# discord/lilliput

Hardware: NVIDIA H100
Metric: images_per_sec_1080p_jpeg_to_256x256_jpeg_q85 (higher is better)
Workload: dtype u8

## Files before the change

### lilliput_b200/csrc/abi_opencv.cu

```cuda
#include <algorithm>
#include <cstring>
#include <memory>
#include <mutex>
#include <new>
#include <string>
#include <vector>

#include "common.cuh"
#include "kernels.cuh"
#include "lp_opencv.h"

namespace lp {

thread_local long g_launches = 0;

static std::once_flag g_dev_once;
static int g_dev_status = LP_ERR_CUDA;

int ensure_device() {
    std::call_once(g_dev_once, [] {
        int n = 0;
        cudaError_t e = cudaGetDeviceCount(&n);
        if (e != cudaSuccess || n == 0) {
            fprintf(stderr,
// ... 99 lines not shown
    m->type = type;
    m->step = row;
    m->dev_off = 0;
    m->dev_step = row;
    m->is_view = false;
    m->dev_valid = true;
    m->host_valid = false;
    return LP_OK;
}

struct Decoder {
    const uint8_t* data = nullptr;
    size_t len = 0;
    JpegHeader jpeg;
    PngHeader png;
    bool is_png = false;
    bool header_ok = false;
    std::string description;
};

struct Encoder {
    std::string ext;
    Mat* dst = nullptr;
};

static int sync_stream() {
    LP_CUDA_OK(cudaStreamSynchronize(thread_stream()));
    return LP_OK;
}

static int decode_jpeg_into(const Decoder* d, Mat* m) {
    const JpegHeader& h = d->jpeg;
    if (!h.supported && !h.multiscan) {
        fprintf(stderr, "[lilliput_b200] JPEG variant not supported on the device path (sampling layout)\n");
        return LP_ERR_UNSUPPORTED;
    }
    std::vector<JpegScanDesc> scans;
    std::vector<JpegHuffSet> sets(1);
    int nscans = 0, nsets = 1;
    if (h.multiscan) {
        scans.resize(kMultiscanMaxScans);
        sets.resize(kMultiscanMaxSets);
        int rc = jpeg_parse_scans(d->data, d->len, h, scans.data(), (int)scans.size(), &nscans, sets.data(),
                                  (int)sets.size(), &nsets);
        if (rc) return rc;
        const size_t visits = jpeg_multiscan_visits(h, scans.data(), nscans);
        if (visits > kMultiscanMaxVisits) {
            fprintf(stderr, "[lilliput_b200] multi-scan JPEG: %zu block visits over %d scans exceed the serial decoder's budget\n",
                    visits, nscans);
            return LP_ERR_UNSUPPORTED;
        }
    } else {
        jpeg_build_huff_set(h, &sets[0]);
        if (h.restart_interval) {
            scans.resize(1);
            jpeg_baseline_scan(h, &scans[0]);
            nscans = 1;
        }
    }
    const bool parallel = nscans == 0;
    cudaStream_t st = thread_stream();
    JpegDecodeItem it;
    memset(&it, 0, sizeof(it));
    it.scan_off = 0;
    it.scan_len = (uint32_t)h.scan_length;
    it.table_set = 0;
    it.restart_interval = h.restart_interval;
    const uint32_t total_blocks = jpeg_decode_item(h, &it);
    uint32_t tiles = 0;
    const uint32_t blocks = jpeg_item_set_window(&it, 0, 0, h.width, h.height, false, &tiles);
    if (!parallel) {
        it.restart_interval = 0;
        it.table_set = 0;
        it.nscans = (uint32_t)nscans;
    }

    uint8_t* scratch = nullptr;
    const size_t upload_len = parallel ? h.scan_length : d->len;
    const size_t scan_bytes = round_up(upload_len + 16, (size_t)256);
    const size_t sets_b = round_up(sizeof(JpegHuffSet) * (size_t)nsets, (size_t)256);
    const size_t scans_b = round_up(sizeof(JpegScanDesc) * (size_t)nscans + 16, (size_t)256);
    const size_t coef_bytes = round_up((size_t)blocks * 64 * sizeof(int16_t), (size_t)256);
    const size_t clean_b = parallel ? round_up(huff_clean_bytes(h.scan_length), (size_t)256) : 0;
    const size_t states_b = parallel ? round_up(2 * huff_nsub(h.scan_length) * 8, (size_t)256) : 0;
    const size_t nslots_b = parallel ? round_up(2 * huff_nsub(h.scan_length) * 4, (size_t)256) : 0;
    const size_t dcdiff_b = parallel ? round_up((size_t)total_blocks * 2, (size_t)256) : 0;
    const size_t total = 1024 + sets_b + scan_bytes + coef_bytes + clean_b + states_b + nslots_b +
                         dcdiff_b + scans_b;
    LP_CUDA_OK(cudaMallocAsync(&scratch, total, st));
    JpegDecodeItem* d_item = reinterpret_cast<JpegDecodeItem*>(scratch);
    JpegHuffSet* d_hs = reinterpret_cast<JpegHuffSet*>(scratch + 1024);
    uint8_t* d_scan = scratch + 1024 + sets_b;
    int16_t* d_coef = reinterpret_cast<int16_t*>(d_scan + scan_bytes);
    uint8_t* d_clean = reinterpret_cast<uint8_t*>(d_coef) + coef_bytes;
    uint8_t* d_states = d_clean + clean_b;
    uint8_t* d_nslots = d_states + states_b;
    uint8_t* d_dcdiff = d_nslots + nslots_b;
    JpegScanDesc* d_scans = reinterpret_cast<JpegScanDesc*>(d_dcdiff + dcdiff_b);
    LP_CUDA_OK(cudaMemcpyAsync(d_item, &it, sizeof(it), cudaMemcpyHostToDevice, st));
    LP_CUDA_OK(cudaMemcpyAsync(d_hs, sets.data(), sizeof(JpegHuffSet) * nsets, cudaMemcpyHostToDevice, st));
    if (parallel) {
        LP_CUDA_OK(cudaMemcpyAsync(d_scan, d->data + h.scan_offset, h.scan_length, cudaMemcpyHostToDevice, st));
    } else {
        LP_CUDA_OK(cudaMemcpyAsync(d_scans, scans.data(), sizeof(JpegScanDesc) * nscans, cudaMemcpyHostToDevice, st));
        LP_CUDA_OK(cudaMemcpyAsync(d_scan, d->data, d->len, cudaMemcpyHostToDevice, st));
    }
    JpegDecodeBatch b;
    b.items = d_item;
    b.tables = d_hs;
    b.scan = d_scan;
    b.coef = d_coef;
    b.frames = m->dptr();
    b.n = 1;
    b.max_tiles_per_image = (int)tiles;
    b.clean = d_clean;
    b.states = d_states;
    b.nslots = reinterpret_cast<uint32_t*>(d_nslots);
    b.dcdiff = reinterpret_cast<int16_t*>(d_dcdiff);
    if (!parallel) {
        b.n_multiscan = 1;
        b.scans = d_scans;
    }
    int rc = jpeg_decode_launch(b, st, nullptr);
    JpegDecodeItem back;
    if (!rc) {
        LP_CUDA_OK(cudaMemcpyAsync(&back, d_item, sizeof(back), cudaMemcpyDeviceToHost, st));
        rc = sync_stream();
    }
    cudaFreeAsync(scratch, st);
    if (rc) return rc;
    return back.status == 0 ? LP_OK : LP_ERR_DECODING_FAILED;
}

static int decode_png_into(const Decoder* d, Mat* m) {
    const PngHeader& h = d->png;
    if (h.idat_total < 2) return LP_ERR_DECODING_FAILED;
    cudaStream_t st = thread_stream();
    PngDecodeItem it;
    png_decode_item(h, (uint32_t)m->dev_step, &it);
    std::vector<uint8_t> z(h.idat_total + 16, 0);
    size_t o = 0;
    for (const PngSegment& sgm : h.idat) {
        memcpy(z.data() + o, d->data + sgm.offset, sgm.length);
        o += sgm.length;
    }
    const size_t zb = round_up(z.size(), (size_t)256);
    const size_t rawb = round_up((size_t)it.raw_total + 16, (size_t)256);
    uint8_t* scratch = nullptr;
    LP_CUDA_OK(cudaMallocAsync(&scratch, 4096 + zb + rawb, st));
    PngDecodeItem* d_item = reinterpret_cast<PngDecodeItem*>(scratch);
    uint8_t* d_z = scratch + 4096;
    uint8_t* d_raw = d_z + zb;
    static_assert(sizeof(PngDecodeItem) <= 4096, "item fits its slot");
    LP_CUDA_OK(cudaMemcpyAsync(d_item, &it, sizeof(it), cudaMemcpyHostToDevice, st));
    LP_CUDA_OK(cudaMemcpyAsync(d_z, z.data(), z.size(), cudaMemcpyHostToDevice, st));
    PngDecodeBatch b;
    b.items = d_item;
    b.z = d_z;
    b.raw = d_raw;
    b.frames = m->dptr();
    b.n = 1;
    b.max_width = h.width;
    b.max_height = h.height;
    int rc = png_decode_launch(b, st);
    PngDecodeItem back;
    if (!rc) {
        LP_CUDA_OK(cudaMemcpyAsync(&back, d_item, sizeof(back), cudaMemcpyDeviceToHost, st));
// ... 612 lines not shown
```

### lilliput_b200/csrc/batch.cu

```cuda
#include <algorithm>
#include <cstring>
#include <map>
#include <string>
#include <thread>
#include <unordered_map>
#include <utility>
#include <vector>

#include "common.cuh"
#include "kernels.cuh"
#include "lilliput_host.hpp"

using namespace lp;

static constexpr int kScansPerImage = 16, kSetsPerImage = 10;

namespace lp {
size_t batch_multiscan_pool_bytes(size_t n) {
    return ((kSetsPerImage * n + kMultiscanMaxSets) * sizeof(JpegHuffSet) +
            (kScansPerImage * n + kMultiscanMaxScans) * sizeof(JpegScanDesc));
}
}

struct lp_batch {
// ... 180 lines not shown
        b->crop_y = y0;
        b->crop_w = x1 - x0;
        b->crop_h = y1 - y0;
    }
    const int slots = jpeg_huff_parallel_slots();
    b->chunk = cfg->chunk > 0 ? cfg->chunk : (slots > 0 ? 3 * slots : 512);
    b->first_chunk = slots > 0 ? std::min(slots, b->chunk) : b->chunk / 2;
    b->pipe_chunk = (cfg->chunk > 0 || slots <= 0) ? b->chunk : std::min(b->chunk, 2 * slots);
    b->chunk = std::min(b->chunk, cfg->max_images);
    b->pipe_chunk = std::max(1, std::min(b->pipe_chunk, b->chunk));
    b->max_chunks = ceil_div(cfg->max_images, b->pipe_chunk) + 3;
    const size_t mcus = (size_t)ceil_div(b->W, 8) * ceil_div(b->H, 8);
    b->max_blocks_alloc = mcus * 3 + 4 * ((size_t)ceil_div(b->W, 8) + ceil_div(b->H, 8)) + 16;
    const size_t max_blocks = b->max_blocks_alloc;
    b->frame_bytes = (size_t)b->W * b->H * 3;
    b->resized_bytes = (size_t)b->out_w * b->out_h * 3;
    if (b->orient) {
        b->resized_bytes = std::max(b->resized_bytes, (size_t)b->out_w2 * b->out_h2 * 3);
        b->oriented_bytes = round_up((size_t)std::max(b->crop_w * b->crop_h, b->crop2_w * b->crop2_h) * 3, (size_t)256);
    }
    const size_t N = cfg->max_images;
    auto fail = [&]() -> lp_batch* { batch_free(b); return nullptr; };
#define BALLOC(ptr, bytes)                                                                      \
    if (dev_arena) {                                                                            \
        const size_t need_ = round_up((size_t)(bytes), (size_t)256);                            \
        if (dev_used + need_ > dev_bytes) return fail();                                        \
        (ptr) = reinterpret_cast<decltype(ptr)>(dev_arena + dev_used);                          \
        dev_used += need_;                                                                      \
    } else if (cudaMalloc(&(ptr), (bytes)) != cudaSuccess) {                                    \
        fprintf(stderr, "[lilliput_b200] lp_batch_create: cudaMalloc(%zu) failed\n", (size_t)(bytes)); \
        return fail();                                                                          \
    }
#define HALLOC(ptr, bytes)                                                                      \
    if (host_arena) {                                                                           \
        const size_t need_ = round_up((size_t)(bytes), (size_t)256);                            \
        if (host_used + need_ > host_bytes) return fail();                                      \
        (ptr) = reinterpret_cast<decltype(ptr)>(host_arena + host_used);                        \
        host_used += need_;                                                                     \
    } else if (cudaMallocHost(&(ptr), (bytes)) != cudaSuccess) {                                \
        return fail();                                                                          \
    }
    if (cudaStreamCreateWithFlags(&b->st, cudaStreamNonBlocking) != cudaSuccess) return fail();
    if (cudaStreamCreateWithFlags(&b->st_h2d, cudaStreamNonBlocking) != cudaSuccess) return fail();
    if (cudaStreamCreateWithFlags(&b->st_d2h, cudaStreamNonBlocking) != cudaSuccess) return fail();
    BALLOC(b->d_scan, cfg->max_in_bytes + 16 * N + 4096);
    BALLOC(b->d_items, N * sizeof(JpegDecodeItem));
    b->max_tables = (int)N;
    if (b->multiscan) {
        b->max_tables += (int)(kSetsPerImage * N) + kMultiscanMaxSets;
        b->max_scans = kScansPerImage * N + kMultiscanMaxScans;
        BALLOC(b->d_scans, b->max_scans * sizeof(JpegScanDesc));
        BALLOC(b->d_masks, (size_t)b->chunk * max_blocks * sizeof(uint64_t));
    }
    BALLOC(b->d_tables, (size_t)b->max_tables * sizeof(JpegHuffSet));
    BALLOC(b->d_coef, (size_t)b->chunk * max_blocks * 64 * sizeof(int16_t));
    BALLOC(b->d_frames, (size_t)b->chunk * (b->orient ? round_up(b->frame_bytes, (size_t)256) : b->frame_bytes) + 256);
    if (b->geoms.empty()) {
        BALLOC(b->d_resized, N * b->resized_bytes + 256);
    } else {
        size_t all = 0;
        for (const BatchGeom& g : b->geoms) {
            b->geom_off.push_back(all);
            all += N * ((size_t)g.out_w * g.out_h * 3);
        }
        BALLOC(b->d_resized, all + 256);
    }
    if (!b->resize_only) {
        size_t enc = jpeg_encode_scratch_bytes(b->out_w, b->out_h, 3, b->chunk, cfg->out_cap, b->progressive);
        if (b->orient)
            enc = std::max(enc, jpeg_encode_scratch_bytes(b->out_w2, b->out_h2, 3, b->chunk, cfg->out_cap, b->progressive));
        for (int c = 0; c < (b->gray ? 2 : 0); c++)
            enc = std::max(enc, jpeg_encode_scratch_bytes(c ? b->out_w2 : b->out_w, c ? b->out_h2 : b->out_h, 1, b->chunk,
                                                          cfg->out_cap, b->progressive));
        BALLOC(b->d_enc_scratch, enc);
    }
    if (b->orient) {
        BALLOC(b->d_oriented, (size_t)b->chunk * b->oriented_bytes);
        BALLOC(b->d_jobs, N * sizeof(OrientJob));
    }
    if (b->orient || b->gray) {
        BALLOC(b->d_index, N * sizeof(int));
    }
    BALLOC(b->d_clean, cfg->max_in_bytes + 64 * N + 4096);
    b->state_cap = (cfg->max_in_bytes / 128 + 2 * N + 16) * 2;
    BALLOC(b->d_states, b->state_cap * 8);
    BALLOC(b->d_nslots, b->state_cap * 4);
    BALLOC(b->d_dcdiff, (size_t)b->chunk * max_blocks * sizeof(int16_t));
    if (!b->resize_only) {
        BALLOC(b->d_out, N * cfg->out_cap);
        BALLOC(b->d_out_len, N * sizeof(uint32_t));
    }
#undef BALLOC
    if (!b->resize_only) {
        HALLOC(b->h_out, N * cfg->out_cap);
        HALLOC(b->h_out_len, N * sizeof(uint32_t));
    }
    HALLOC(b->h_items_back, N * sizeof(JpegDecodeItem));
    if (!b->resize_only) {
        HALLOC(b->h_off, (N + (size_t)b->max_chunks + 8) * sizeof(unsigned long long));
    }
#undef HALLOC
    b->ev.resize((size_t)b->max_chunks * 6);
    b->ev_h2d.resize(b->max_chunks);
    b->ev_d2h.resize(b->max_chunks);
    for (auto& e : b->ev)
        if (cudaEventCreate(&e) != cudaSuccess) return fail();
    for (auto& e : b->ev_h2d)
        if (cudaEventCreateWithFlags(&e, cudaEventDisableTiming) != cudaSuccess) return fail();
    for (auto& e : b->ev_d2h)
        if (cudaEventCreateWithFlags(&e, cudaEventDisableTiming) != cudaSuccess) return fail();
    b->items.resize(N);
    b->parse_status.resize(N);
    b->file_dev_off.resize(N);
    if (b->orient) {
        b->jobs.resize(N);
    }
    if (b->orient || b->gray) b->index.resize(N);
    b->arena_dev_used = dev_used;
    b->arena_host_used = host_used;
    return b;
}

void lp::batch_arena_used(const lp_batch* b, size_t* dev_bytes, size_t* host_bytes) {
    *dev_bytes = b->arena_dev_used;
    *host_bytes = b->arena_host_used;
}

extern "C" void lp_batch_destroy(lp_batch* b) {
    if (!b) return;
    DeviceGuard dev_guard(b->cfg.device);
    cudaDeviceSynchronize();
    batch_free(b);
}

static int table_set_lookup(lp_batch* b, const JpegHeader& h);
static int table_set_for(lp_batch* b, const JpegHeader& h) {
    if (b->last_table_idx >= 0 && !memcmp(h.huff_present, b->last_present, sizeof(h.huff_present)) &&
        !memcmp(h.huff_bits, b->last_bits, sizeof(h.huff_bits)) && !memcmp(h.huff_vals, b->last_vals, sizeof(h.huff_vals)))
        return b->last_table_idx;
    const int found = table_set_lookup(b, h);
    if (found >= 0) {
        memcpy(b->last_present, h.huff_present, sizeof(h.huff_present));
        memcpy(b->last_bits, h.huff_bits, sizeof(h.huff_bits));
        memcpy(b->last_vals, h.huff_vals, sizeof(h.huff_vals));
        b->last_table_idx = found;
    }
    return found;
}

static int table_set_lookup(lp_batch* b, const JpegHeader& h) {
    std::string key;
    for (int tc = 0; tc < 2; tc++)
        for (int th = 0; th < 4; th++) {
            key.push_back((char)h.huff_present[tc][th]);
            if (h.huff_present[tc][th]) {
                key.append((const char*)h.huff_bits[tc][th], 17);
                key.append((const char*)h.huff_vals[tc][th], 256);
            }
        }
    auto it = b->table_index.find(key);
    if (it != b->table_index.end()) return it->second;
    if ((int)b->tables.size() >= b->max_tables) return -1;
    JpegHuffSet hs;
    jpeg_build_huff_set(h, &hs);
    b->tables.push_back(hs);
    int idx = (int)b->tables.size() - 1;
    b->table_index[key] = idx;
// ... 77 lines not shown
                uint32_t tiles = 0;
                const uint32_t blocks = jpeg_item_set_window(&it, x0, y0, x1, y1, true, &tiles);
                blocks_of[k - i0] = blocks;
                tiles_of[k - i0] = tiles;
                total_of[k - i0] = total_blocks;
                if (blocks > b->max_blocks_alloc || total_blocks > b->max_blocks_alloc)
                    rc = LP_ERR_UNSUPPORTED;
            }
            b->parse_status[k] = rc;
            it.status = rc ? -1 : 0;
        }
    };
    const int nthreads = cnt >= 256 ? 4 : 1;
    if (nthreads == 1) {
        pass1(i0, i0 + cnt);
    } else {
        std::vector<std::thread> pool;
        const int per = ceil_div(cnt, nthreads);
        for (int t = 1; t < nthreads; t++)
            pool.emplace_back(pass1, std::min(i0 + cnt, i0 + t * per), std::min(i0 + cnt, i0 + (t + 1) * per));
        pass1(i0, std::min(i0 + cnt, i0 + per));
        for (auto& th : pool) th.join();
    }
    lp_batch::ChunkLayout lay;
    lay.ordinal = ordinal;
    size_t rotated_window_bytes = 0;
    for (int k = i0; k < i0 + cnt; k++) {
        if (b->parse_status[k]) continue;
        const JpegDecodeItem& it = b->items[k];
        lay.blocks = std::max(lay.blocks, blocks_of[k - i0]);
        lay.tiles = std::max(lay.tiles, tiles_of[k - i0]);
        lay.total_blocks = std::max(lay.total_blocks, total_of[k - i0]);
        if (class_of[k - i0] % 3) rotated_window_bytes = std::max(rotated_window_bytes, (size_t)it.win_stride * it.win_h);
        if (!b->layout_known) {
            JpegDecodeItem a = it;
            jpeg_item_set_window(&a, b->crop_x, b->crop_y, b->crop_x + b->crop_w, b->crop_y + b->crop_h, true, nullptr);
            b->win_w = a.win_w;
            b->win_h = a.win_h;
            b->win_x0 = a.win_x0;
            b->frame_bytes = (size_t)jpeg_window_row_bytes(a.win_x0, a.win_w, a.width, 3) * a.win_h;
            b->gray_row_bytes = jpeg_window_row_bytes(a.win_x0, a.win_w, a.width, 1);
            b->layout_known = true;
        }
    }
    lay.frame_stride = rotated_window_bytes > b->frame_bytes ? round_up(rotated_window_bytes, (size_t)256) : b->frame_bytes;
    b->blocks = std::max(b->blocks, lay.blocks);
    b->total_blocks = std::max(b->total_blocks, lay.total_blocks);
    b->chunk_layout[i0] = lay;
    for (int k = i0; k < i0 + cnt; k++) {
        if (b->parse_status[k]) continue;
        JpegDecodeItem& it = b->items[k];
        const int slot = k - i0;
        if (!ms_scans[slot].empty()) {
            const std::vector<JpegScanDesc>& sc = ms_scans[slot];
            const std::vector<JpegHeader>& sets = ms_sets[slot];
            std::vector<int> global(sets.size(), -1);
            bool fits = b->scans.size() + sc.size() <= b->max_scans;
            for (size_t q = 0; q < sets.size() && fits; q++) fits = (global[q] = table_set_for(b, sets[q])) >= 0;
            if (!fits) {
                b->parse_status[k] = LP_ERR_UNSUPPORTED;
                it.status = -1;
                continue;
            }
            it.table_set = (uint32_t)b->scans.size();
            it.nscans = (uint32_t)sc.size();
            for (JpegScanDesc d : sc) {
                d.table_set = global[d.table_set];
                b->scans.push_back(d);
            }
            it.scan_off = b->file_dev_off[k];
            it.coef_off = (uint64_t)slot * lay.blocks * 64;
            it.frame_off = (uint64_t)slot * lay.frame_stride;
            it.dcdiff_off = (uint64_t)slot * lay.total_blocks;
            b->chunk_layout[i0].n_multiscan++;
            continue;
        }
        const int ts = table_set_for(b, hdr[k - i0]);
        if (ts < 0) {
            b->parse_status[k] = LP_ERR_UNSUPPORTED;
            it.status = -1;
            continue;
        }
        it.table_set = (uint32_t)ts;
        size_t state_need = 2 * huff_nsub(it.scan_len);
        if (it.restart_interval) {
            const uint32_t mcus = (uint32_t)it.mcus_x * it.mcus_y;
            const uint32_t nint = (mcus + (uint32_t)it.restart_interval - 1) / (uint32_t)it.restart_interval;
            it.clean_len = nint;
            state_need = std::max(state_need, (size_t)nint + 2);
            if (b->state_off + state_need > b->state_cap) {
                b->parse_status[k] = LP_ERR_UNSUPPORTED;
                it.status = -1;
                continue;
            }
            for (uint32_t q = 0; q < nint; q++) b->chunk_layout[i0].rst_work.push_back(make_uint2((unsigned)slot, q));
        }
        it.scan_off = b->file_dev_off[k] + hdr[k - i0].scan_offset;
        it.coef_off = (uint64_t)slot * lay.blocks * 64;
        it.frame_off = (uint64_t)slot * lay.frame_stride;
        it.dcdiff_off = (uint64_t)slot * lay.total_blocks;
        it.clean_off = b->clean_off;
        it.state_off = b->state_off;
        b->clean_off += huff_clean_bytes(it.scan_len);
        b->state_off += state_need;
    }
    if (!b->index.empty()) {
        lp_batch::ChunkLayout& cl = b->chunk_layout[i0];
        int* idx = b->index.data() + i0;
        int at = 0, rotated = 0;
        for (int s = 0; s < 6; s++) {
            const int c = s % 3;
            for (int k = i0; k < i0 + cnt; k++) {
                const int cls = b->parse_status[k] ? 0 : class_of[k - i0];
                if (cls != s) continue;
                idx[at++] = k - i0;
                cl.n_class[s]++;
                if (!c) continue;
                const JpegDecodeItem& it = b->items[k];
                OrientJob& j = b->jobs[i0 + rotated++];
                j.src_off = it.frame_off;
                j.dst_off = (uint64_t)(k - i0) * b->oriented_bytes;
                j.src_stride = it.win_stride;
                j.o = hdr[k - i0].orientation;
                j.cx = c == 1 ? b->crop_x : b->crop2_x;
                j.cy = c == 1 ? b->crop_y : b->crop2_y;
                j.cw = c == 1 ? b->crop_w : b->crop2_w;
                j.ch = c == 1 ? b->crop_h : b->crop2_h;
                j.win_x0 = it.win_x0;
                j.win_y0 = it.win_y0;
            }
        }
    }
    return LP_OK;
}

static int batch_upload_files(lp_batch* b, const uint8_t* const* in, const size_t* in_len, int i0, int cnt,
                              cudaStream_t st) {
    int i = i0;
    while (i < i0 + cnt) {
        int j = i;
        size_t run = in_len[i];
        while (j + 1 < i0 + cnt && in[j + 1] == in[j] + in_len[j]) { j++; run += in_len[j]; }
        LP_CUDA_OK(cudaMemcpyAsync(b->d_scan + b->file_dev_off[i], in[i], run, cudaMemcpyHostToDevice, st));
        i = j + 1;
    }
    return LP_OK;
}

static int batch_upload_items(lp_batch* b, int i0, int cnt, cudaStream_t st) {
    LP_CUDA_OK(cudaMemcpyAsync(b->d_items + i0, b->items.data() + i0, (size_t)cnt * sizeof(JpegDecodeItem),
                               cudaMemcpyHostToDevice, st));
    const auto lay = b->chunk_layout.find(i0);
    if (lay != b->chunk_layout.end()) {
        const int* nc = lay->second.n_class;
        const int rotated = nc[1] + nc[2] + nc[4] + nc[5];
        if (lay->second.mapped(cnt))
            LP_CUDA_OK(cudaMemcpyAsync(b->d_index + i0, b->index.data() + i0, (size_t)cnt * sizeof(int), cudaMemcpyHostToDevice, st));
        if (rotated)
            LP_CUDA_OK(cudaMemcpyAsync(b->d_jobs + i0, b->jobs.data() + i0, (size_t)rotated * sizeof(OrientJob),
                                       cudaMemcpyHostToDevice, st));
    }
    if (b->tables.size() > b->tables_uploaded) {
        LP_CUDA_OK(cudaMemcpyAsync(b->d_tables + b->tables_uploaded, b->tables.data() + b->tables_uploaded,
                                   (b->tables.size() - b->tables_uploaded) * sizeof(JpegHuffSet),
                                   cudaMemcpyHostToDevice, st));
        b->tables_uploaded = b->tables.size();
    }
// ... 465 lines not shown
```

### lilliput_b200/csrc/jpeg_huff_parallel.cu

```cuda
#include <cstdlib>

#include "common.cuh"
#include "kernels.cuh"

namespace lp {

__device__ unsigned long long g_huff_phase[8];
#define LP_PHASE_MARK(k)                                             \
    do {                                                             \
        if (threadIdx.x == 0) {                                      \
            const long long now_ = clock64();                        \
            atomicAdd(&g_huff_phase[k], (unsigned long long)(now_ - s_tphase)); \
            s_tphase = now_;                                         \
        }                                                            \
    } while (0)

constexpr uint32_t kMinSubBits = 1024;
constexpr uint32_t kSubPerThread = 1;
#ifndef LP_HUFF_THREADS
#define LP_HUFF_THREADS 384
#endif
constexpr int kHuffThreads = LP_HUFF_THREADS;
constexpr int kUnstuffThreads = 512;

__constant__ uint8_t c_zigzag_p[64] = {0,  1,  8,  16, 9,  2,  3,  10, 17, 24, 32, 25, 18, 11, 4,  5,
                                       12, 19, 26, 33, 40, 48, 41, 34, 27, 20, 13, 6,  7,  14, 21, 28,
                                       35, 42, 49, 56, 57, 50, 43, 36, 29, 22, 15, 23, 30, 37, 44, 51,
                                       58, 59, 52, 45, 38, 31, 39, 46, 53, 60, 61, 54, 47, 55, 62, 63};


template <int THREADS>
__device__ __forceinline__ uint32_t block_excl_scan(uint32_t v, uint32_t* total, uint32_t* warp_sums) {
    const int lane = threadIdx.x & 31, wid = threadIdx.x >> 5;
    uint32_t inc = v;
#pragma unroll
    for (int o = 1; o < 32; o <<= 1) {
        const uint32_t t = __shfl_up_sync(0xffffffffu, inc, o);
        if (lane >= o) inc += t;
    }
    if (lane == 31) warp_sums[wid] = inc;
    __syncthreads();
    if (wid == 0) {
        uint32_t s = lane < THREADS / 32 ? warp_sums[lane] : 0;
#pragma unroll
        for (int o = 1; o < 32; o <<= 1) {
            const uint32_t t = __shfl_up_sync(0xffffffffu, s, o);
            if (lane >= o) s += t;
        }
        if (lane < THREADS / 32) warp_sums[lane] = s;
    }
    __syncthreads();
    const uint32_t base = wid ? warp_sums[wid - 1] : 0;
    *total = warp_sums[THREADS / 32 - 1];
    __syncthreads();
    return base + inc - v;
}


__global__ void __launch_bounds__(kUnstuffThreads)
    jpeg_unstuff_kernel(JpegDecodeItem* items, const uint8_t* scan, uint8_t* clean) {
    __shared__ uint32_t warp_sums[kUnstuffThreads / 32];
    __shared__ uint32_t s_end;
    __shared__ __align__(16) uint8_t stage[kUnstuffThreads * 16 + 16];
    JpegDecodeItem& it = items[blockIdx.x];
    const uint8_t* src = scan + it.scan_off;
    const uint32_t len = it.scan_len;
    uint8_t* dst = clean + it.clean_off;
    const int tid = threadIdx.x, lane = tid & 31;
    if (it.restart_interval != 0 || it.nscans != 0) return;
    if (it.status != 0) {
        if (tid == 0) it.clean_len = 0;
        return;
    }
    if (tid == 0) s_end = len;
    __syncthreads();
    const uint32_t mis = (uint32_t)(reinterpret_cast<uintptr_t>(src) & 15);
    const uint8_t* abase = src - mis;
    uint32_t carry = 0;
    uint32_t end = len;
    constexpr uint32_t kTile = kUnstuffThreads * 16;
    for (uint32_t t0 = 0; t0 < mis + end; t0 += kTile) {
        const uint32_t aoff = t0 + (uint32_t)tid * 16;
        const int64_t i0 = (int64_t)aoff - (int64_t)mis;
        uint4 w = make_uint4(0, 0, 0, 0);
        if (aoff < mis + len + 16) w = *reinterpret_cast<const uint4*>(abase + aoff);
        uint32_t prev = __shfl_up_sync(0xffffffffu, w.w >> 24, 1);
        uint32_t next = __shfl_down_sync(0xffffffffu, w.x & 0xffu, 1);
        if (lane == 0) prev = i0 > 0 ? src[i0 - 1] : 0;
        if (lane == 31) next = (i0 + 16 < (int64_t)len) ? src[i0 + 16] : 0xD9u;
        const uint32_t ws[4] = {w.x, w.y, w.z, w.w};
        uint32_t m00[4], mff[4];
#pragma unroll
        for (int q = 0; q < 4; q++) {
            m00[q] = __vcmpeq4(ws[q], 0u);
            mff[q] = __vcmpeq4(ws[q], 0xFFFFFFFFu);
        }
        const uint32_t prev_ff = prev == 0xFFu ? 0xFFu : 0u, next_00 = next == 0x00u ? 0xFF000000u : 0u;
        uint32_t drop16 = 0, mark16 = 0;
#pragma unroll
        for (int q = 0; q < 4; q++) {
            const uint32_t pff = (mff[q] << 8) | (q ? mff[q - 1] >> 24 : prev_ff);
// ... 230 lines not shown
            set_tables();
            if (--blocks_left == 0) break;
            dcp++;
        }
    }
    if (WRITE && bad) *status = -3;
    p = limit - (uint32_t)bits_left;
    phase = (blk << 6) | z;
    nslots = closed * 64 + z - z_start;
}

template <bool WRITE>
__device__ __forceinline__ void decode_span(const HuffShared& hs, const uint8_t* s, uint32_t& p, uint32_t limit,
                                            uint32_t end_bits, uint32_t& phase, uint32_t& nslots, int nb,
                                            uint64_t pos, uint64_t total_slots, const JpegDecodeItem* it,
                                            int16_t* coef, int16_t* dcdiff, int* status) {
    if (hs.two_tables)
        decode_span_t<WRITE, true>(hs, s, p, limit, end_bits, phase, nslots, nb, pos, total_slots, it, coef, dcdiff, status);
    else
        decode_span_t<WRITE, false>(hs, s, p, limit, end_bits, phase, nslots, nb, pos, total_slots, it, coef, dcdiff, status);
}

__device__ __forceinline__ void dc_prefix_pass(const JpegDecodeItem& it, int16_t* coef, const int16_t* dcdiff, int nb,
                                               uint32_t* warp_sums) {
    const int tid = threadIdx.x;
    constexpr int kDcRun = 8;
    const uint32_t mcus_x = (uint32_t)it.mcus_x;
    const int roi_mx0 = it.roi_mx0, roi_my0 = it.roi_my0, roi_mcx = it.roi_mcx, roi_mcy = it.roi_mcy;
    int koff = 0;
    for (int c = 0; c < it.ncomp; c++) {
        const uint32_t bpc = (uint32_t)(it.h[c] * it.v[c]);
        const uint32_t nblk = mcus_x * (uint32_t)it.mcus_y * bpc;
        const int16_t* dsrc = dcdiff + koff;
        int16_t* cdst = coef + it.coef_off + (size_t)koff * 64;
        uint32_t dc_before = 0;
        for (uint32_t base = 0; base < nblk; base += kHuffThreads * kDcRun) {
            const uint32_t j0 = base + (uint32_t)tid * kDcRun;
            const uint32_t mcu0 = j0 / bpc, kk0 = j0 % bpc;
            int d[kDcRun];
            uint32_t sum = 0;
            {
                uint32_t mcu = mcu0, kk = kk0;
#pragma unroll
                for (int r = 0; r < kDcRun; r++) {
                    d[r] = j0 + r < nblk ? dsrc[(size_t)mcu * nb + kk] : 0;
                    sum += (uint32_t)d[r];
                    if (++kk == bpc) {
                        kk = 0;
                        mcu++;
                    }
                }
            }
            uint32_t total;
            const uint32_t ex = block_excl_scan<kHuffThreads>(sum, &total, warp_sums);
            uint32_t run = dc_before + ex;
            dc_before += total;
            uint32_t mcu = mcu0, kk = kk0;
            int mx = (int)(mcu0 % mcus_x) - roi_mx0, my = (int)(mcu0 / mcus_x) - roi_my0;
#pragma unroll
            for (int r = 0; r < kDcRun; r++) {
                run += (uint32_t)d[r];
                if (j0 + r < nblk && (unsigned)mx < (unsigned)roi_mcx && (unsigned)my < (unsigned)roi_mcy)
                    cdst[(((size_t)my * roi_mcx + mx) * nb + kk) * 64] = (int16_t)(int)run;
                if (++kk == bpc) {
                    kk = 0;
                    mcu++;
                    if (++mx == (int)mcus_x - roi_mx0) {
                        mx = -roi_mx0;
                        my++;
                    }
                }
            }
        }
        koff += (int)bpc;
    }
}

#ifndef LP_HUFF_MIN_CTAS
#define LP_HUFF_MIN_CTAS 4
#endif
__global__ void __launch_bounds__(kHuffThreads, LP_HUFF_MIN_CTAS)
    jpeg_huff_sync_kernel(JpegDecodeItem* items, const JpegHuffSet* tables, const uint8_t* clean,
                          SubState* states_all, uint32_t* nslots_all, int16_t* coef, int16_t* dcdiff_all,
                          uint32_t sub_per_thread) {
    __shared__ HuffShared hs;
    __shared__ uint32_t warp_sums[kHuffThreads / 32];
    __shared__ uint32_t s_carry;
    __shared__ int s_status;
    JpegDecodeItem& it = items[blockIdx.x];
    const int tid = threadIdx.x;
    if (it.status != 0 || it.restart_interval != 0 || it.nscans != 0) return;
    __shared__ long long s_tphase;
    __shared__ unsigned long long s_bits[2];
    if (tid == 0) s_tphase = clock64();
    {
        const JpegHuffSet* g = tables + it.table_set;
        for (int i = tid; i < 8 * 18; i += kHuffThreads) (&hs.maxcode[0][0])[i] = (&g->maxcode[0][0])[i];
        for (int i = tid; i < 8 * 17; i += kHuffThreads) (&hs.valoffset[0][0])[i] = (&g->valoffset[0][0])[i];
        for (int i = tid; i < 8 * 256; i += kHuffThreads) (&hs.vals[0][0])[i] = (&g->vals[0][0])[i];
        for (int i = tid; i < 4 * (1 << kDcBits); i += kHuffThreads) (&hs.dc_look[0][0])[i] = (&g->look[0][0])[i];
        for (int i = tid; i < 4 * (1 << kAcBits); i += kHuffThreads) (&hs.ac_look[0][0])[i] = 0;
        if (tid < 64) hs.zz[tid] = c_zigzag_p[tid];
        if (tid == 0) {
            int k = 0;
            for (int c = 0; c < it.ncomp; c++)
                for (int j = 0; j < it.h[c] * it.v[c]; j++, k++) {
                    hs.blk_dc[k] = (uint8_t)it.td[c];
                    hs.blk_ac[k] = (uint8_t)it.ta[c];
                    hs.blk_comp[k] = (uint8_t)c;
                    hs.blk_bx[k] = (uint8_t)(j % it.h[c]);
                    hs.blk_by[k] = (uint8_t)(j / it.h[c]);
                }
            const int nfirst = it.h[0] * it.v[0];
            bool two = true;
            for (int b = 0; b < k; b++) {
                const int ref = b < nfirst ? 0 : nfirst;
                if (hs.blk_dc[b] != hs.blk_dc[ref] || hs.blk_ac[b] != hs.blk_ac[ref]) two = false;
            }
            const int rest = nfirst < k ? nfirst : 0;
            hs.two_tables = two;
            hs.n_first = (uint32_t)nfirst;
            hs.dcb_first = (uint32_t)__cvta_generic_to_shared(&hs.dc_look[hs.blk_dc[0]][0]);
            hs.acb_first = (uint32_t)__cvta_generic_to_shared(&hs.ac_look[hs.blk_ac[0]][0]);
            hs.dcb_rest = (uint32_t)__cvta_generic_to_shared(&hs.dc_look[hs.blk_dc[rest]][0]);
            hs.acb_rest = (uint32_t)__cvta_generic_to_shared(&hs.ac_look[hs.blk_ac[rest]][0]);
            s_status = 0;
            s_carry = 0;
            s_bits[0] = s_bits[1] = 0;
        }
    }
    __syncthreads();
    {
        const JpegHuffSet* g = tables + it.table_set;
        for (int i = tid; i < 4 * (1 << kAcBits); i += kHuffThreads) {
            const int t = i >> kAcBits, idx = i & ((1 << kAcBits) - 1);
            uint16_t e = g->look[4 + t][idx >> (kAcBits - 9)];
            if (!e) {
                for (int len = 10; len <= kAcBits; len++) {
                    const int code = idx >> (kAcBits - len);
                    if (code <= hs.maxcode[4 + t][len]) {
                        e = (uint16_t)((len << 8) | hs.vals[4 + t][(code + hs.valoffset[4 + t][len]) & 0xFF]);
                        break;
                    }
                }
            }
            hs.ac_look[t][idx] = e;
        }
        for (int i = tid; i < 4 * kHuffLongPrefixes * 16; i += kHuffThreads)
            (&hs.ac_sub[0][0])[i] = (&g->long_sub[0][0][0])[i];
    }
    __syncthreads();
    if (tid < 4 * kHuffLongPrefixes) {
        const uint32_t pfx = (tables + it.table_set)->long_prefix[tid / kHuffLongPrefixes][tid % kHuffLongPrefixes];
        if (pfx < (1u << kAcBits)) hs.ac_look[tid / kHuffLongPrefixes][pfx] = (uint16_t)(0x8000u | (uint32_t)tid);
    }
    __syncthreads();
    int nb = 0;
    for (int c = 0; c < it.ncomp; c++) nb += it.h[c] * it.v[c];
    const uint8_t* s = clean + it.clean_off;
    const uint32_t total_bits = it.clean_len * 8u;
    uint32_t kSubBits = (total_bits + kHuffThreads * sub_per_thread - 1) / (kHuffThreads * sub_per_thread);
    kSubBits = max(kMinSubBits, (kSubBits + 31u) & ~31u);
    const uint32_t nsub = (total_bits + kSubBits - 1) / kSubBits;
    SubState* st = states_all + it.state_off;
    uint32_t* ns = nslots_all + it.state_off;
    uint32_t* list_a = reinterpret_cast<uint32_t*>(st + nsub);
    uint32_t* list_b = list_a + nsub;
    const uint64_t total_slots = (uint64_t)it.mcus_x * it.mcus_y * nb * 64;
    int16_t* dcdiff = dcdiff_all + it.dcdiff_off;

    LP_PHASE_MARK(0);
    for (uint32_t i = tid; i < nsub; i += kHuffThreads) {
        uint32_t p = i * kSubBits, phase = 0, n = 0;
        const uint32_t limit = min((i + 1) * kSubBits, total_bits);
        decode_span<false>(hs, s, p, limit, total_bits, phase, n, nb, 0, 0, nullptr, nullptr, nullptr, nullptr);
        atomicAdd(&s_bits[1], (unsigned long long)(p - i * kSubBits));
        st[i] = SubState{p, phase};
        ns[i] = n;
    }
    __syncthreads();
    LP_PHASE_MARK(1);
    uint32_t* cur_list = list_a;
    uint32_t* nxt_list = list_b;
    uint32_t cur_count = nsub > 0 ? nsub - 1 : 0;
    bool first_round = true;
    uint32_t rounds = 0;
    while (cur_count > 0) {
        rounds++;
        if (tid == 0) s_carry = 0;
        __syncthreads();
        for (uint32_t k = tid; k < cur_count; k += kHuffThreads) {
            const uint32_t i = first_round ? k + 1 : cur_list[k];
            const uint64_t in64 = *reinterpret_cast<volatile uint64_t*>(&st[i - 1]);
            const SubState in{(uint32_t)in64, (uint32_t)(in64 >> 32)};
            const SubState old = st[i];
            uint32_t p = in.p, phase = in.phase, n = 0;
            const uint32_t limit = min((i + 1) * kSubBits, total_bits);
            if (p < limit) {
                decode_span<false>(hs, s, p, limit, total_bits, phase, n, nb, 0, 0, nullptr, nullptr, nullptr, nullptr);
                atomicAdd(&s_bits[0], (unsigned long long)(p - in.p));
            }
            ns[i] = n;
            if (p != old.p || phase != old.phase) {
                *reinterpret_cast<volatile uint64_t*>(&st[i]) = ((uint64_t)phase << 32) | p;
                if (i + 1 < nsub) nxt_list[atomicAdd(&s_carry, 1u)] = i + 1;
            }
        }
        __syncthreads();
        cur_count = s_carry;
        __syncthreads();
        uint32_t* t = cur_list;
        cur_list = nxt_list;
        nxt_list = t;
        first_round = false;
    }
    if (tid == 0) {
        it.pad_ = rounds;
        atomicAdd(&g_huff_phase[6], s_bits[0]);
        atomicAdd(&g_huff_phase[7], s_bits[1]);
    }
    LP_PHASE_MARK(2);
    SubState* cur = st;
    uint64_t slots_before = 0;
    for (uint32_t base = 0; base < nsub; base += kHuffThreads) {
        const uint32_t i = base + tid;
        const uint32_t v = i < nsub ? ns[i] : 0;
        uint32_t total;
        const uint32_t ex = block_excl_scan<kHuffThreads>(v, &total, warp_sums);
        const uint64_t pos = slots_before + ex;
        slots_before += total;
        if (i < nsub) {
            uint32_t p = i == 0 ? 0u : cur[i - 1].p;
            uint32_t phase = i == 0 ? 0u : cur[i - 1].phase;
            uint32_t n = 0;
            const uint32_t limit = min((i + 1) * kSubBits, total_bits);
            int status = 0;
            if (pos < total_slots &&
                (uint32_t)(pos % ((uint64_t)nb * 64)) != ((phase >> 6) * 64 + (phase & 63)))
                status = -3;
            if (!status && p < limit)
                decode_span<true>(hs, s, p, limit, total_bits, phase, n, nb, pos, total_slots, &it, coef, dcdiff, &status);
            if (status) s_status = status;
        }
    }
    if (tid == 0 && slots_before < total_slots) s_status = -3;
    __syncthreads();
    if (s_status) {
        if (tid == 0) it.status = s_status;
        return;
    }
    LP_PHASE_MARK(3);
    dc_prefix_pass(it, coef, dcdiff, nb, warp_sums);
    LP_PHASE_MARK(4);
    if (tid == 0) atomicAdd(&g_huff_phase[5], 1ull);
}



int jpeg_huff_phase_clocks(unsigned long long out[8], int reset) {
    LP_CUDA_OK(cudaDeviceSynchronize());
    LP_CUDA_OK(cudaMemcpyFromSymbol(out, g_huff_phase, sizeof(unsigned long long) * 8));
    if (reset) {
        unsigned long long z[8] = {0, 0, 0, 0, 0, 0, 0, 0};
        LP_CUDA_OK(cudaMemcpyToSymbol(g_huff_phase, z, sizeof(z)));
    }
    return LP_OK;
}

int jpeg_huff_parallel_slots() {
    int dev = 0, sms = 0, per_sm = 0;
    if (cudaGetDevice(&dev) != cudaSuccess) return 0;
    cudaDeviceGetAttribute(&sms, cudaDevAttrMultiProcessorCount, dev);
    cudaOccupancyMaxActiveBlocksPerMultiprocessor(&per_sm, jpeg_huff_sync_kernel, kHuffThreads, 0);
    return sms * per_sm;
}

int jpeg_huff_parallel_launch(const JpegHuffParallelArgs& a, cudaStream_t st) {
    if (a.n <= 0) return LP_OK;
    static const uint32_t spt = getenv("LP_HUFF_SPT") ? (uint32_t)atoi(getenv("LP_HUFF_SPT")) : kSubPerThread;
    jpeg_unstuff_kernel<<<a.n, kUnstuffThreads, 0, st>>>(a.items, a.scan, a.clean);
    g_launches++;
    LP_CUDA_OK(cudaGetLastError());
    jpeg_huff_sync_kernel<<<a.n, kHuffThreads, 0, st>>>(a.items, a.tables, a.clean,
                                                       reinterpret_cast<SubState*>(a.states), a.nslots, a.coef,
                                                       a.dcdiff, spt);
    g_launches++;
    LP_CUDA_OK(cudaGetLastError());
    return LP_OK;
}

}
```

Before: 53440.

## Add lead-in decoding to parallel Huffman subsequences to cut sync rounds

Each subsequence now starts decoding a fraction (6/16) of a subsequence width before its nominal boundary, so it is likely already synchronized when it reaches that boundary. The entry state it computed is stored in a new array, and only subsequences whose stored entry state differs from their predecessor's exit state go on the initial fix-up list. Later rounds skip any subsequence whose incoming state matches the recorded one. This aims to cut the number and cost of resynchronization rounds, in exchange for extra decode work in the first pass and a larger state buffer (3x instead of 2x).

```diff
diff --git a/lilliput_b200/csrc/abi_opencv.cu b/lilliput_b200/csrc/abi_opencv.cu
--- a/lilliput_b200/csrc/abi_opencv.cu
+++ b/lilliput_b200/csrc/abi_opencv.cu
@@ -205,7 +205,7 @@
     const size_t scans_b = round_up(sizeof(JpegScanDesc) * (size_t)nscans + 16, (size_t)256);
     const size_t coef_bytes = round_up((size_t)blocks * 64 * sizeof(int16_t), (size_t)256);
     const size_t clean_b = parallel ? round_up(huff_clean_bytes(h.scan_length), (size_t)256) : 0;
-    const size_t states_b = parallel ? round_up(2 * huff_nsub(h.scan_length) * 8, (size_t)256) : 0;
+    const size_t states_b = parallel ? round_up(3 * huff_nsub(h.scan_length) * 8, (size_t)256) : 0;
     const size_t nslots_b = parallel ? round_up(2 * huff_nsub(h.scan_length) * 4, (size_t)256) : 0;
     const size_t dcdiff_b = parallel ? round_up((size_t)total_blocks * 2, (size_t)256) : 0;
     const size_t total = 1024 + sets_b + scan_bytes + coef_bytes + clean_b + states_b + nslots_b +
diff --git a/lilliput_b200/csrc/batch.cu b/lilliput_b200/csrc/batch.cu
--- a/lilliput_b200/csrc/batch.cu
+++ b/lilliput_b200/csrc/batch.cu
@@ -286,7 +286,7 @@
         BALLOC(b->d_index, N * sizeof(int));
     }
     BALLOC(b->d_clean, cfg->max_in_bytes + 64 * N + 4096);
-    b->state_cap = (cfg->max_in_bytes / 128 + 2 * N + 16) * 2;
+    b->state_cap = (cfg->max_in_bytes / 128 + 2 * N + 16) * 3;
     BALLOC(b->d_states, b->state_cap * 8);
     BALLOC(b->d_nslots, b->state_cap * 4);
     BALLOC(b->d_dcdiff, (size_t)b->chunk * max_blocks * sizeof(int16_t));
@@ -530,7 +530,7 @@
             continue;
         }
         it.table_set = (uint32_t)ts;
-        size_t state_need = 2 * huff_nsub(it.scan_len);
+        size_t state_need = 3 * huff_nsub(it.scan_len);
         if (it.restart_interval) {
             const uint32_t mcus = (uint32_t)it.mcus_x * it.mcus_y;
             const uint32_t nint = (mcus + (uint32_t)it.restart_interval - 1) / (uint32_t)it.restart_interval;
diff --git a/lilliput_b200/csrc/jpeg_huff_parallel.cu b/lilliput_b200/csrc/jpeg_huff_parallel.cu
--- a/lilliput_b200/csrc/jpeg_huff_parallel.cu
+++ b/lilliput_b200/csrc/jpeg_huff_parallel.cu
@@ -17,6 +17,7 @@
 
 constexpr uint32_t kMinSubBits = 1024;
 constexpr uint32_t kSubPerThread = 1;
+constexpr uint32_t kLeadIn16 = 6;
 #ifndef LP_HUFF_THREADS
 #define LP_HUFF_THREADS 384
 #endif
@@ -413,7 +414,7 @@
 __global__ void __launch_bounds__(kHuffThreads, LP_HUFF_MIN_CTAS)
     jpeg_huff_sync_kernel(JpegDecodeItem* items, const JpegHuffSet* tables, const uint8_t* clean,
                           SubState* states_all, uint32_t* nslots_all, int16_t* coef, int16_t* dcdiff_all,
-                          uint32_t sub_per_thread) {
+                          uint32_t sub_per_thread, uint32_t leadin16) {
     __shared__ HuffShared hs;
     __shared__ uint32_t warp_sums[kHuffThreads / 32];
     __shared__ uint32_t s_carry;
@@ -494,36 +495,54 @@
     kSubBits = max(kMinSubBits, (kSubBits + 31u) & ~31u);
     const uint32_t nsub = (total_bits + kSubBits - 1) / kSubBits;
     SubState* st = states_all + it.state_off;
+    SubState* en = st + nsub;
     uint32_t* ns = nslots_all + it.state_off;
-    uint32_t* list_a = reinterpret_cast<uint32_t*>(st + nsub);
+    uint32_t* list_a = reinterpret_cast<uint32_t*>(en + nsub);
     uint32_t* list_b = list_a + nsub;
     const uint64_t total_slots = (uint64_t)it.mcus_x * it.mcus_y * nb * 64;
     int16_t* dcdiff = dcdiff_all + it.dcdiff_off;
+    const uint32_t lead = (uint32_t)((uint64_t)kSubBits * leadin16 / 16);
 
     LP_PHASE_MARK(0);
     for (uint32_t i = tid; i < nsub; i += kHuffThreads) {
-        uint32_t p = i * kSubBits, phase = 0, n = 0;
-        const uint32_t limit = min((i + 1) * kSubBits, total_bits);
-        decode_span<false>(hs, s, p, limit, total_bits, phase, n, nb, 0, 0, nullptr, nullptr, nullptr, nullptr);
-        atomicAdd(&s_bits[1], (unsigned long long)(p - i * kSubBits));
+        const uint32_t p0 = i * kSubBits;
+        const uint32_t start = i == 0 ? 0u : p0 - lead;
+        uint32_t p = start, phase = 0, n = 0;
+#pragma unroll 1
+        for (uint32_t seg = i == 0 ? 1u : 0u; seg < 2; seg++) {
+            const uint32_t limit = seg ? min(p0 + kSubBits, total_bits) : p0;
+            if (seg) en[i] = SubState{p, phase};
+            n = 0;
+            if (p < limit)
+                decode_span<false>(hs, s, p, limit, total_bits, phase, n, nb, 0, 0, nullptr, nullptr, nullptr, nullptr);
+        }
+        atomicAdd(&s_bits[1], (unsigned long long)(p - start));
         st[i] = SubState{p, phase};
         ns[i] = n;
     }
     __syncthreads();
     LP_PHASE_MARK(1);
-    uint32_t* cur_list = list_a;
-    uint32_t* nxt_list = list_b;
-    uint32_t cur_count = nsub > 0 ? nsub - 1 : 0;
-    bool first_round = true;
+    for (uint32_t i = tid + 1; i < nsub; i += kHuffThreads) {
+        const SubState e = en[i], l = st[i - 1];
+        if (e.p != l.p || e.phase != l.phase) list_a[atomicAdd(&s_carry, 1u)] = i;
+    }
+    __syncthreads();
+    uint32_t cur_count = s_carry;
     uint32_t rounds = 0;
+    __syncthreads();
     while (cur_count > 0) {
+        const uint32_t* cur_list = rounds & 1 ? list_b : list_a;
+        uint32_t* nxt_list = rounds & 1 ? list_a : list_b;
         rounds++;
         if (tid == 0) s_carry = 0;
         __syncthreads();
         for (uint32_t k = tid; k < cur_count; k += kHuffThreads) {
-            const uint32_t i = first_round ? k + 1 : cur_list[k];
+            const uint32_t i = cur_list[k];
             const uint64_t in64 = *reinterpret_cast<volatile uint64_t*>(&st[i - 1]);
             const SubState in{(uint32_t)in64, (uint32_t)(in64 >> 32)};
+            const SubState was = en[i];
+            if (in.p == was.p && in.phase == was.phase) continue;
+            en[i] = in;
             const SubState old = st[i];
             uint32_t p = in.p, phase = in.phase, n = 0;
             const uint32_t limit = min((i + 1) * kSubBits, total_bits);
@@ -540,10 +559,6 @@
         __syncthreads();
         cur_count = s_carry;
         __syncthreads();
-        uint32_t* t = cur_list;
-        cur_list = nxt_list;
-        nxt_list = t;
-        first_round = false;
     }
     if (tid == 0) {
         it.pad_ = rounds;
@@ -609,12 +624,14 @@
 int jpeg_huff_parallel_launch(const JpegHuffParallelArgs& a, cudaStream_t st) {
     if (a.n <= 0) return LP_OK;
     static const uint32_t spt = getenv("LP_HUFF_SPT") ? (uint32_t)atoi(getenv("LP_HUFF_SPT")) : kSubPerThread;
+    static const uint32_t leadin16 =
+        getenv("LP_HUFF_LEADIN") ? min(16u, (uint32_t)atoi(getenv("LP_HUFF_LEADIN"))) : kLeadIn16;
     jpeg_unstuff_kernel<<<a.n, kUnstuffThreads, 0, st>>>(a.items, a.scan, a.clean);
     g_launches++;
     LP_CUDA_OK(cudaGetLastError());
     jpeg_huff_sync_kernel<<<a.n, kHuffThreads, 0, st>>>(a.items, a.tables, a.clean,
                                                        reinterpret_cast<SubState*>(a.states), a.nslots, a.coef,
-                                                       a.dcdiff, spt);
+                                                       a.dcdiff, spt, leadin16);
     g_launches++;
     LP_CUDA_OK(cudaGetLastError());
     return LP_OK;
```

Result: no change. 53490, median of 6 (+0.1%).
